# tumaer/lagrangebench

Measured on AMD Instinct MI355X. Metric: rollout particle-steps/sec, higher is better.
Workload: dtype f32 (GEMMs as fp16 hi/lo split products, fp32 accumulate)

## Files before the change

### lagrangebench_amd/build.py

```python
from __future__ import annotations

import os
import subprocess
import sys
from concurrent.futures import ThreadPoolExecutor

HERE = os.path.dirname(os.path.abspath(__file__))
CSRC = os.path.join(HERE, "csrc")
LIB = os.path.join(CSRC, "liblbhip.so")
SOURCES = ["lb_api.hip", "lb_neighbor.hip", "lb_state.hip", "lb_gns.hip", "lb_gns_weights.hip", "lb_edge16.hip", "lb_segnn.hip", "lb_segnn_gen.hip", "lb_segnn_msg.hip", "lb_segnn_node.hip", "lb_sinkhorn.hip", "lb_edge16v.hip", "lb_edge16w.hip", "lb_node16s.hip", "lb_gns_generic.hip", "lb_msplit.hip", "lb_train.hip", "lb_egnn.hip", "lb_painn.hip", "lb_train_input.hip"]
HEADERS = ["lb_internal.h", "lb_device.h", "lb_f16x2.h", "lb_segnn_dev.h", "lb_features.h", "lb_msplit.h", "lb_msplit_dev.h", "lb_lin32.h", "lb_train_segnn.h", "lb_train_egnn.h", os.path.join("..", "..", "include", "lbhip.h")]
FLAGS = ["-O3", "-std=c++17", "--offload-arch=gfx950", "-fPIC", "-ffp-contract=off",
         "-Wall", "-Wno-unused-function"]
EXTRA_FLAGS = {"lb_edge16v.hip": ["-fno-slp-vectorize"],
               "lb_edge16w.hip": ["-fno-slp-vectorize", "-mllvm", "-pragma-unroll-threshold=10000000"], "lb_node16s.hip": ["-fno-slp-vectorize"],
               "lb_gns_generic.hip": ["-fno-slp-vectorize"], "lb_segnn_msg.hip": ["-fno-slp-vectorize"], "lb_segnn_node.hip": ["-fno-slp-vectorize"], "lb_msplit.hip": ["-fno-slp-vectorize"]}


def _rocm_root() -> str:
    root = os.environ.get("ROCM_PATH")
    if root and os.path.isdir(root):
        return root
    try:
        out = subprocess.run(["hipconfig", "--rocmpath"], capture_output=True, text=True, timeout=30).stdout.strip()
        if out and os.path.isdir(out):
            return out
    except (OSError, subprocess.SubprocessError):
        pass
    return "/opt/rocm"


def _hipcc() -> str:
    for c in (os.path.join(_rocm_root(), "bin", "hipcc"), "/opt/rocm/bin/hipcc", "hipcc"):
        if os.path.exists(c) or c == "hipcc":
            return c
    raise RuntimeError("hipcc not found")


def _stale(target: str, deps) -> bool:
    if not os.path.exists(target):
        return True
    t = os.path.getmtime(target)
    return any(os.path.getmtime(d) > t for d in deps)

# ... 33 lines not shown
```

### lagrangebench_amd/csrc/lb_api.hip

```cpp
#include <cstddef>
#include <stdarg.h>
#include <stdio.h>
#include <stdlib.h>
#include <string.h>

#include <algorithm>
#include <cmath>

#include <initializer_list>
#include <tuple>

#include "lb_internal.h"
#include "lb_msplit.h"

thread_local std::string g_lb_err;

int lb_fail(int code, const char* fmt, ...) {
  char buf[1024];
  va_list ap;
  va_start(ap, fmt);
  vsnprintf(buf, sizeof(buf), fmt, ap);
  va_end(ap);
  g_lb_err = buf;
  return code;
// ... 85 lines not shown
  return (cls >= 0 && cls < LB_T_COUNT) ? k_timer_names[cls] : "";
}
extern "C" int lb_timer_get(lb_engine* e, int32_t cls, double* ms_out, int64_t* launches_out) {
  if (!e || cls < 0 || cls >= LB_T_COUNT) return lb_fail(LB_ERR_ARG, "bad timer class");
  lb_timers_collect(e);
  if (ms_out) *ms_out = e->t_ms[cls];
  if (launches_out) *launches_out = e->t_n[cls];
  return LB_OK;
}


extern "C" int lb_engine_create(const lb_case_desc* d, void* hip_stream, lb_engine** out) {
  if (!d || !out) return lb_fail(LB_ERR_ARG, "null argument");
  if (d->dim != 2 && d->dim != 3) return lb_fail(LB_ERR_ARG, "dim must be 2 or 3 (got %d)", d->dim);
  if (d->n_particles < 1 || d->batch < 1 || d->isl < 2)
    return lb_fail(LB_ERR_ARG, "need n_particles>=1, batch>=1, isl>=2");
  if (!(d->r_cutoff > 0)) return lb_fail(LB_ERR_ARG, "r_cutoff must be > 0");
  if ((int64_t)d->n_particles * d->batch > (int64_t)1 << 30)
    return lb_fail(LB_ERR_ARG, "B*N too large for int32 node ids");
  lb_engine* e = new lb_engine();
  e->desc = *d;
  e->stream = (hipStream_t)hip_stream;
  e->BN = (int64_t)d->n_particles * d->batch;
  e->timers_on = false;
  for (int i = 0; i < LB_T_COUNT; ++i) e->t_ms[i] = 0, e->t_n[i] = 0;
  {
    const char* f = getenv("LB_FUSED_AGG");
    e->fused_agg = (f && f[0] == '0') ? 0 : 1;
    const char* m = getenv("LB_MATH");
    e->f16x2 = (m && !strcmp(m, "f32")) ? 0 : 1;
    e->math_auto = m ? 0 : 1;
    const char* gf = getenv("LB_GUARD");
    e->guard_full = (gf && !strcmp(gf, "full")) ? 1 : 0;
    e->guard_sampled = (gf && !strcmp(gf, "sampled")) ? 1 : 0;
  }
  lb_geom& g = e->g;
  memset(&g, 0, sizeof(g));
  g.dim = d->dim;
  g.N = d->n_particles;
  g.B = d->batch;
  g.isl = d->isl;
  g.periodic = d->periodic != 0;
  g.has_bound = d->has_bound != 0;
  g.has_vel_mag = d->has_vel_mag != 0;
  g.force_kind = d->force_kind;
  g.force_axis = d->force_axis;
  g.f32 = d->geometry_f32 != 0;
  auto R = [&](double x) { return g.f32 ? (double)(float)x : x; };
  g.rc = R(d->r_cutoff);
  g.rc2 = R(d->r_cutoff * d->r_cutoff);
  bool use_cells = true;
  for (int k = 0; k < d->dim; ++k) {
    const float b32 = (float)d->box[k];
    if (!((float)d->r_cutoff < b32 / 3.0f)) use_cells = false;
  }
  g.use_cell_list = use_cells;
  g.ncells = 1;
  for (int k = 0; k < 3; ++k) {
    g.ncell[k] = 1;
    g.cell_size[k] = 1.0;
    g.box[k] = k < d->dim ? R(d->box[k]) : 1.0;
    g.half_box[k] = g.box[k] * 0.5;
    g.vel_mean[k] = R(d->vel_mean[k]);
    g.vel_std[k] = R(d->vel_std[k]);
    g.acc_mean[k] = R(d->acc_mean[k]);
    g.acc_std[k] = R(d->acc_std[k]);
// ... 698 lines not shown
```

### lagrangebench_amd/csrc/lb_gns.hip

```cpp
#include <stdio.h>

#include <algorithm>
#include <stdlib.h>

#include "lb_device.h"
#include "lb_msplit.h"

#define MFMA(a, b, c) __builtin_amdgcn_mfma_f32_32x32x2f32((a), (b), (c), 0, 0, 0)

void lb_pack_weight(const float* w, int K, int M, int Kpad, int Mpad, float* out) {
  const int NKQ = Kpad / 8, NMB = Mpad / 32;
  for (int kq = 0; kq < NKQ; ++kq)
    for (int mb = 0; mb < NMB; ++mb)
      for (int lane = 0; lane < 64; ++lane)
        for (int j = 0; j < 4; ++j) {
          const int k = 8 * kq + 4 * (lane >> 5) + j;
          const int m = 32 * mb + (lane & 31);
          out[(((size_t)kq * NMB + mb) * 64 + lane) * 4 + j] =
              (k < K && m < M) ? w[(size_t)k * M + m] : 0.f;
        }
}

template <int NKQ, int NMB, int PF = 1, typename LD>
__device__ __forceinline__ void lb_gemm(LD ld, const f32x4 (&v)[NKQ], f32x16 (&acc)[NMB]) {
// ... 300 lines not shown
    a.tile_shift = 4;
    a.row_ptr = e->row_ptr;
    a.part = e->part;
    if (ms) {
      lb_nms_args m{};
      m.ctrl = e->ctrl;
      m.n_rows = BN;
      m.xin = xin;
      m.agg = e->agg;
      m.row_ptr = e->row_ptr;
      m.part = e->part;
      m.fused = e->fused_agg;
      m.nlat = e->nlat;
      m.w = w.ms;
      m.b0 = a.b0;
      m.b1 = a.b1;
      m.ln_s = a.ln_s;
      m.ln_o = a.ln_o;
      m.bp = a.bp;
      m.psr = e->psr;
      if (dec) {
        m.bd0 = g->dec.b0;
        m.bd1 = g->dec.b1;
        m.dec_unscale = g->dec_unscale;
        m.acc_out = e->acc;
        m.out_dim = g->desc.out_dim;
        if (e->integ_job.on && g->desc.out_dim == e->g.dim) {
          m.integ = e->integ_job;
          e->integ_done = true;
        }
      }
      return lbk_node_ms(e, m, kq / 4, with_agg, resid, proj, dec);
    }
    if (e->f16x2)
      return lbk_node16s(e, a, w.w0_16h, w.w1_16h, proj ? g->proc_edge[next].proj_w_h2 : nullptr, kq / 4, with_agg ? 4 : 0,
                         resid);
    if (with_agg)
      hipLaunchKernelGGL((k_node_mlp<16, 16, true>), dim3(ntile_n), dim3(64), 0, s, a);
    else if (kq == 4)
      hipLaunchKernelGGL((k_node_mlp<4, 0, false>), dim3(ntile_n), dim3(64), 0, s, a);
    else if (kq == 8)
      hipLaunchKernelGGL((k_node_mlp<8, 0, false>), dim3(ntile_n), dim3(64), 0, s, a);
    else if (kq == 12)
      hipLaunchKernelGGL((k_node_mlp<12, 0, false>), dim3(ntile_n), dim3(64), 0, s, a);
    else
      hipLaunchKernelGGL((k_node_mlp<16, 0, false>), dim3(ntile_n), dim3(64), 0, s, a);
    return LB_OK;
  };

  lb_tic(e, LB_T_ENC_NODE);
  rc = node_mlp(g->enc_node, e->xnode, g->kq_node, false, false, 0, ms_en);
  lb_toc(e);
  if (rc) return rc;

  bool decoded = false;
  lb_tic(e, LB_T_ENC_EDGE);
  if (ms_ee) {
    lb_ems_args m{};
    m.ctrl = e->ctrl;
    m.efeat = e->efeat;
    m.elat = e->elat;
    m.w = g->enc_edge.ms;
    m.b0 = g->enc_edge.b0;
    m.b1 = g->enc_edge.b1;
    m.ln_s = g->enc_edge.ln_s;
    m.ln_o = g->enc_edge.ln_o;
    rc = lbk_edge_enc_ms(e, m);
  } else {
    lb_edge16_args b{};
// ... 34 lines not shown
    } else {
      lb_edge16_args b{};
      b.ctrl = e->ctrl;
      b.senders = e->senders;
      b.receivers = e->receivers;
      b.elat = e->elat;
      b.msg = e->msg;
      b.psr = e->psr;
      b.w0p = e->f16x2 ? pe.w0_16h : pe.w0_16;
      b.w1p = e->f16x2 ? pe.w1_16h : pe.w1_16;
      b.b1 = pe.b1;
      b.ln_s = pe.ln_s;
      b.ln_o = pe.ln_o;
      b.fused = e->fused_agg;
      b.row_ptr = e->row_ptr;
      b.agg = e->agg;
      b.part = e->part;
      b.aggpart_bytes = e->aggpart_bytes;
      b.skip_elat_store = skip;
      if (e->f16x2 && e->fused_agg)
        rc = lb_use_edge_w(e) ? lbk_edge16w(e, b) : lbk_edge16v(e, b);
      else
        rc = lbk_edge16(e, b, true, e->f16x2 != 0);
    }
    lb_toc(e);
    if (rc) return rc;
    if (!e->fused_agg) {
      lb_tic(e, LB_T_AGGREGATE);
      rc = lbk_segment_sum(e, e->msg, e->agg, LB_D);
      lb_toc(e);
      if (rc) return rc;
    }
    const bool ms_dec_ok = lb_fused_launches();
    const bool with_dec = ms_pn && ms_dec_ok && k == L - 1 && e->f16x2 && g->desc.out_dim <= 4;
    lb_tic_single(e, LB_T_NODE_MLP);
    rc = node_mlp(g->proc_node[k], e->nlat, 16, true, true, k + 1, ms_pn, with_dec);
    lb_toc(e);
    decoded = with_dec;
    if (rc) return rc;
    if (g->tap)
      LB_HIP(hipMemcpyAsync(g->tap + (size_t)(k + 1) * BN * LB_D, e->nlat, sizeof(float) * BN * LB_D,
                            hipMemcpyDeviceToDevice, s));
  }
  if (decoded) return LB_OK;
  lb_tic(e, LB_T_DECODER);
  rc = lbk_decoder16(e, g);
  lb_toc(e);
  if (rc) return rc;
  LB_HIP(hipGetLastError());
  return LB_OK;
}
```

### lagrangebench_amd/csrc/lb_gns_generic.hip

```cpp
#include <algorithm>
#include <cmath>
#include <cstring>
#include <vector>

#include "lb_f16x2.h"
#include "lb_features.h"

#define MFMA16F(a, b, c) __builtin_amdgcn_mfma_f32_16x16x4f32((a), (b), (c), 0, 0, 0)
#define GD_THREADS 512
#define GD_WAVES 8

struct lb_dense_args {
  const lb_ctrl* ctrl;
  int64_t n_rows;
  const float* x;
  int x_blocked;
  int x_stride, x_width;
  const float* w;
  const float* bias;
  const float* add0;
  const int32_t* idx0;
  const float* add1;
  const int32_t* idx1;
  const float* ln_s;
  const float* ln_o;
  const float* resid;
  int resid_blocked;
  float* out;
  int out_blocked;
  float* out_pre;
  float* acc_out;
  int out_dim;
};

__device__ __forceinline__ void lb_gemm16f(lds_cptr wl, const f32x4 (&v)[8], f32x4 (&acc)[8]) {
  f32x4 a0 = wl[0], a1 = wl[64];
#pragma unroll
  for (int step = 0; step < 32; ++step) {
    f32x4 n0 = a0, n1 = a1;
// ... 125 lines not shown
      bool bad = false;
      for (int d = 0; d < a.out_dim; ++d) bad |= !(fabsf(o[d]) <= 3.0e38f);
      if (bad) lb_raise_math(a.ctrl, LB_MATH_NONFINITE);
    }
  }
}

static int lbk_dense16(lb_engine* e, const lb_dense_args& a, int64_t rows_bound, bool relu_in) {
  const int64_t tiles = std::max<int64_t>(1, (rows_bound + 15) / 16);
  const int grid = (int)std::min<int64_t>(512, (tiles + GD_WAVES - 1) / GD_WAVES);
  if (e->f16x2) {
    if (relu_in)
      hipLaunchKernelGGL((k_dense16<true, true>), dim3(grid), dim3(GD_THREADS), 0, e->stream, a);
    else
      hipLaunchKernelGGL((k_dense16<true, false>), dim3(grid), dim3(GD_THREADS), 0, e->stream, a);
  } else {
    if (relu_in)
      hipLaunchKernelGGL((k_dense16<false, true>), dim3(grid), dim3(GD_THREADS), 0, e->stream, a);
    else
      hipLaunchKernelGGL((k_dense16<false, false>), dim3(grid), dim3(GD_THREADS), 0, e->stream, a);
  }
  LB_HIP(hipGetLastError());
  return LB_OK;
}

struct lb_dec16_args {
  const lb_ctrl* ctrl;
  int64_t n_rows;
  const float* nlat;
  const float* w0;
  const float* b0;
  const float* w1;
  const float* b1;
  float unscale;
  float* acc_out;
  int out_dim;
  lb_integ_job integ;
};

template <bool F16>
__global__ void __launch_bounds__(GD_THREADS, 2) k_decoder16(lb_dec16_args a, lb_geom geom) {
  constexpr int NW1 = F16 ? 512 : 4096;
  __shared__ f32x4 sW[4096 + NW1 + 33];
  const int poisoned = a.ctrl->overflow_step;
  const int step = a.ctrl->step;
  const int tid = threadIdx.x;
  {
    const f32x4* g0 = reinterpret_cast<const f32x4*>(a.w0);
    const f32x4* g1 = reinterpret_cast<const f32x4*>(a.w1);
    for (int i = tid; i < 4096; i += GD_THREADS) sW[i] = g0[i];
    for (int i = tid; i < NW1; i += GD_THREADS) sW[4096 + i] = g1[i];
    if (tid < 32) sW[4096 + NW1 + tid] = reinterpret_cast<const f32x4*>(a.b0)[tid];
    if (tid == 32) sW[4096 + NW1 + 32] = reinterpret_cast<const f32x4*>(a.b1)[0];
  }
  if (poisoned >= 0) return;
  __syncthreads();
  const int ntiles = (int)((a.n_rows + 15) >> 4);
  const int lane = tid & 63, wave = tid >> 6;
  const int n = lane & 15, g = lane >> 4;
  const lds_cptr lw0 = (lds_cptr)sW + lane, lw1 = (lds_cptr)sW + 4096 + lane;
  const lds_cptr lb0 = (lds_cptr)sW + 4096 + NW1 + g;
  const f32x4 b1v = sW[4096 + NW1 + 32];
  const f32x4 zero = {0.f, 0.f, 0.f, 0.f};
  bool probed = false;
  for (int t = blockIdx.x * GD_WAVES + wave; t < ntiles; t += gridDim.x * GD_WAVES) {
    const int64_t row = (int64_t)t * 16 + n;
    const bool valid = row < a.n_rows;
    const int64_t rowc = valid ? row : a.n_rows - 1;
    f32x4 v[8], acc[8];
    lb_integ_in pre{};
    if (a.integ.on && valid && g == 0) pre = lb_integrate_fetch(geom, a.n_rows, a.integ.win, step, a.integ.ptype, row);
    const f32x4* xr = reinterpret_cast<const f32x4*>(a.nlat) + rowc * 32 + g;
#pragma unroll
    for (int mb = 0; mb < 8; ++mb) v[mb] = xr[4 * mb];
#pragma unroll
    for (int mb = 0; mb < 8; ++mb) acc[mb] = lb0[4 * mb];
    f32x4 o = zero;
    if constexpr (F16) {
      if (!probed) {
        lb_range_probe(a.ctrl, v, 8);
        probed = true;
      }
      lb_gemm16v<false, 4>(lw0, v, acc);
      if (t < (int)gridDim.x * GD_WAVES) lb_range_probe(a.ctrl, acc, 8);
#pragma unroll
      for (int p = 0; p < 4; ++p) {
        f32x4 r0, r1;
#pragma unroll
        for (int j = 0; j < 4; ++j) {
          r0[j] = fmaxf(acc[2 * p][j], 0.f);
          r1[j] = fmaxf(acc[2 * p + 1][j], 0.f);
        }
        h8 bh, bl;
        lb_split8v(r0, r1, bh, bl);
        const h8 ah = __builtin_bit_cast(h8, lw1[(p * 2 + 0) * 64]);
        const h8 al = __builtin_bit_cast(h8, lw1[(p * 2 + 1) * 64]);
        o = MFMA16H(al, bh, o);
        o = MFMA16H(ah, bl, o);
        o = MFMA16H(ah, bh, o);
      }
    } else {
      lb_gemm16f(lw0, v, acc);
#pragma unroll
      for (int step = 0; step < 32; ++step) {
        const f32x4 a0 = lw1[(step * 2) * 64];
        o = MFMA16F(a0[0], fmaxf(acc[step >> 2][step & 3], 0.f), o);
      }
    }
    if (valid && g == 0) {
      o = o * a.unscale + b1v;
      reinterpret_cast<f32x4*>(a.acc_out)[row] = o;
      bool bad = false;
      for (int d = 0; d < a.out_dim; ++d) bad |= !(fabsf(o[d]) <= 3.0e38f);
      if (bad) lb_raise_math(a.ctrl, LB_MATH_NONFINITE);
      if (a.integ.on) {
        const float av[4] = {o[0], o[1], o[2], o[3]};
        lb_integrate_body(geom, a.n_rows, a.integ.win, step, a.integ.ptype, av, nullptr, a.integ.traj, a.integ.T,
                          a.integ.pred, a.integ.pred_T, row, &pre);
      }
    }
  }
  if (a.integ.on) {
    __syncthreads();
    if (tid == 0 && atomicAdd(a.integ.blocks_done, 1) == (int)gridDim.x - 1) {
      *a.integ.blocks_done = 0;
      const_cast<lb_ctrl*>(a.ctrl)->step = step + 1;
    }
  }
}

int lbk_decoder16(lb_engine* e, lb_gns* g) {
  lb_dec16_args a{};
  a.ctrl = e->ctrl;
  a.n_rows = e->BN;
  a.nlat = e->nlat;
  a.w0 = e->f16x2 ? g->dec.w0_16h : g->dec.w0_16;
  a.b0 = g->dec.b0;
  a.w1 = e->f16x2 ? g->dec.w1_16h : g->dec.w1_16;
  a.b1 = g->dec.b1;
  a.unscale = e->f16x2 ? g->dec_unscale : 1.f;
  a.acc_out = e->acc;
  a.out_dim = g->desc.out_dim;
  const int64_t tiles = std::max<int64_t>(1, (e->BN + 15) / 16);
  const int grid = (int)std::min<int64_t>(512, (tiles + GD_WAVES - 1) / GD_WAVES);
  if (e->integ_job.on && g->desc.out_dim == e->g.dim) {
    a.integ = e->integ_job;
    e->integ_done = true;
  }
  if (e->f16x2)
    hipLaunchKernelGGL((k_decoder16<true>), dim3(grid), dim3(GD_THREADS), 0, e->stream, a, e->g);
  else
    hipLaunchKernelGGL((k_decoder16<false>), dim3(grid), dim3(GD_THREADS), 0, e->stream, a, e->g);
  LB_HIP(hipGetLastError());
  return LB_OK;
}

int lbk_gns_forward_generic(lb_engine* e, lb_gns* g) {
  hipStream_t s = e->stream;
  const int64_t BN = e->BN;
  const int D = LB_D, L = g->desc.num_mp_steps, nl = g->desc.blocks_per_step;
  int rc;
  if (nl > 1 && g->gen_he_cap < e->e_alloc) {
    LB_HIP(hipStreamSynchronize(s));
    if (g->gen_he) (void)hipFree(g->gen_he);
    g->gen_he = nullptr;
    g->gen_he_cap = 0;
    LB_TRY(lb_alloc(&g->gen_he, (size_t)(e->e_alloc + 32) * D));
    g->gen_he_cap = e->e_alloc;
  }
  const int64_t e_bound = e->e_alloc;
  auto W = [&](const lb_gen_lin& l, int blk) { return e->f16x2 ? l.wh[blk] : l.wf[blk]; };
  auto base_args = [&]() {
    lb_dense_args a{};
    a.ctrl = e->ctrl;
    a.x_stride = D;
    a.x_width = D;
    a.out_dim = g->desc.out_dim;
    return a;
  };
// ... 172 lines not shown
```

### lagrangebench_amd/csrc/lb_gns_weights.hip

```cpp
#include <algorithm>
#include <cmath>
#include <cstdio>
#include <cstring>
#include <utility>
#include <vector>

#include "lb_msplit.h"

struct lb_lin_view {
  const float* w;
  int blocks, rows, out;
  const float* b;
  const float* block(int i) const { return w + (size_t)i * rows * out; }
};
struct lb_mlp_view {
  std::vector<lb_lin_view> lin;
  const float* ln_s = nullptr;
  const float* ln_o = nullptr;
};
struct lb_gns_view {
  const float* embed = nullptr;
  lb_mlp_view enc_node, enc_edge, dec;
  std::vector<lb_mlp_view> proc_edge, proc_node;
};
// ... 165 lines not shown
    put_ms(&m.ms, ms);
  };
  auto proj_piece = [&](const std::vector<float>& wsr) { return std::vector<ms_piece>{{wsr.data(), D, 2 * D, 4, 2, true, 0}}; };

  std::vector<float> wsr, wsr_next;
  if (L) wsr = ws_wr(v.proc_edge[0].lin[0]);
  node_mlp(g->enc_node, v.enc_node, v.enc_node.lin[0].w, v.enc_node.lin[0].rows, dl, g->kq_node * 8,
           L ? proj_piece(wsr) : std::vector<ms_piece>());
  g->proc_edge.resize(L);
  g->proc_node.resize(L);
  for (int k = 0; k < L; ++k) {
    {
      const lb_lin_view &l0 = v.proc_edge[k].lin[0], &l1 = v.proc_edge[k].lin[1];
      lb_mlp_w& m = g->proc_edge[k];
      p32(&m.proj_w, wsr.data(), D, 2 * D, D, 2 * D);
      float* two = st.put(&m.proj_w_h2, (size_t)2 * D * D);
      lb_pack_weight16h(l0.block(0), dl, dl, D, two, D);
      lb_pack_weight16h(l0.block(1), dl, dl, D, two + (size_t)D * D, D);
      memcpy(st.put(&m.proj_b, 2 * D) + D, l0.b, sizeof(float) * dl);
      p16(&m.w0_16, l0.block(2), dl, dl, D);
      p16h(&m.w0_16h, l0.block(2), dl, dl, D);
      p16(&m.w1_16, l1.w, dl, dl, D);
      p16h(&m.w1_16h, l1.w, dl, dl, D);
      vecs(m, v.proc_edge[k], false);
      put_ms(&m.ms, {{l0.block(2), dl, dl, 4, 1, true, 0}, {l1.w, dl, dl, 4, 1, true, 0}});
    }
    const std::vector<float> w0 = lb_lin_padded(v.proc_node[k].lin[0]);
    std::vector<ms_piece> ms = {{d0.w, dl, dl, 4, 1, true, 0}, {d1s.data(), dl, od, 4, 1, true, 2048}};
    if (k + 1 < L) {
      wsr_next = ws_wr(v.proc_edge[k + 1].lin[0]);
      ms = proj_piece(wsr_next);
    }
    node_mlp(g->proc_node[k], v.proc_node[k], w0.data(), 2 * D, D, 2 * D, ms);
    wsr.swap(wsr_next);
  }
}

static void lb_pack_dense(lb_stage& st, const lb_gns_view& v, lb_gns* g) {
  const int D = LB_D, L = g->desc.num_mp_steps;
  auto mlp = [&](lb_gen_mlp& m, const lb_mlp_view& s) {
    m.lin.resize(s.lin.size());
    for (size_t li = 0; li < s.lin.size(); ++li) {
      const lb_lin_view& l = s.lin[li];
      lb_gen_lin& x = m.lin[li];
      st.note_rms(l);
      x.wh.resize(l.blocks);
      x.wf.resize(l.blocks);
      for (int b = 0; b < l.blocks; ++b) {
        lb_pack_weight16h(l.block(b), l.rows, l.out, D, st.put(&x.wh[b], (size_t)D * D), D);
        lb_pack_weight16(l.block(b), l.rows, l.out, D, st.put(&x.wf[b], (size_t)D * D));
      }
      st.put(&x.b, D, l.b, l.out);
    }
    if (s.ln_s) {
      st.put(&m.ln_s, D, s.ln_s, s.lin.back().out);
      st.put(&m.ln_o, D, s.ln_o, s.lin.back().out);
    }
  };
  mlp(g->g_enc_node, v.enc_node);
  mlp(g->g_enc_edge, v.enc_edge);
  g->g_proc_edge.resize(L);
  g->g_proc_node.resize(L);
  for (int k = 0; k < L; ++k) {
    mlp(g->g_proc_edge[k], v.proc_edge[k]);
    mlp(g->g_proc_node[k], v.proc_node[k]);
  }
// ... 73 lines not shown
```

### lagrangebench_amd/csrc/lb_internal.h

```cpp
#pragma once
#include <cstdlib>
#include <hip/hip_ext.h>
#include <hip/hip_runtime.h>
#include <stdint.h>

#include <string>
#include <vector>

#include "../../include/lbhip.h"

#define LB_MAX_STENCIL_CAND 2048
#define LB_MAX_ROW 256
#define LB_MAX_ROW_DENSE 4096
#define LB_TILE 32
#define LB_D 128
#define LB_PAD_TYPE (-1)

typedef float f32x4 __attribute__((ext_vector_type(4)));
typedef float f32x16 __attribute__((ext_vector_type(16)));

struct lb_ctrl {
  int32_t step;
  int32_t overflow_step;
  int32_t n_edges_total;
// ... 116 lines not shown
  unsigned long long* nl_wg_sum = nullptr;
  int32_t* row_ptr;
  int32_t* scan_part;
  double* cpos;
  int64_t cell_slots = 0;
  bool nl_dense = false;
  int32_t row_cap = 0;
  int32_t maxd;
  int32_t* tmp_send;
  float* tmp_feat;
  double* tmp_feat64;
  int32_t* senders;
  int32_t* receivers;
  float* efeat;
  double* efeat64;
  int32_t* overflow;
  int32_t* nedges_b;

  float* xnode;
  float* nlat;
  float* agg;
  float* psr;
  float* elat;
  float* msg;
  float* part;
  int64_t aggpart_bytes = 0;
  int fused_agg;
  int f16x2;
  int math_auto;
  int guard_sampled;
  int math_fallbacks = 0;
  int debug_guard_step = -1;
  int debug_guard_flags = 0;
  int guard_full;
  float* acc;
  const void* bound_model = nullptr;

  bool timers_on;
  std::vector<lb_timer_rec> trecs;
  bool ext_armed = false, ext_used = false;
  std::vector<hipEvent_t> epool;
  double t_ms[LB_T_COUNT];
  int64_t t_n[LB_T_COUNT];
};

struct lb_mlp_w {
  const float* b0;
  const float* b1;
  const float* ln_s;
  const float* ln_o;
  const float* w0;
  const float* w1;
  const float* w0_16;
  const float* w1_16;
  const float* w0_16h;
  const float* w1_16h;
  const float* ms;
  const float* proj_w;
  const float* proj_w_h2;
  const float* proj_b;
};

struct lb_edge16_args {
  const lb_ctrl* ctrl;
  const int32_t* senders;
  const int32_t* receivers;
  const float* efeat;
  float* elat;
  float* elat_out;
  float* msg;
  const float* psr;
  const float* w0p;
  const float* b0;
  const float* w1p;
  const float* b1;
  const float* ln_s;
  const float* ln_o;
  int fused;
  const int32_t* row_ptr;
  float* agg;
  float* part;
  int64_t aggpart_bytes;
  int reverse;
  int skip_elat_store;
};

struct lb_node_args {
  const lb_ctrl* ctrl;
  int64_t n_rows;
  const float* xin;
  const float* agg;
  float* nlat;
  const float* w0p;
// ... 142 lines not shown
int lbk_sgg_forward(lb_engine* e, lb_sgg* m);

void lb_sg_msg_image(const float* ws0, const float* wv0, const float* b0, const float* ws1,
                     const float* wv1, const float* b1, float* out);
int lb_sg_msg_image_floats(void);
int lbk_sg_message(lb_engine* e, const float* f, const float* image, float* agg, float* part, int64_t out_bytes,
                   bool finish);
void lb_sg_upd_image(const float* ws0, const float* wv0, const float* b0, const float* ws1,
                     const float* wv1, const float* b1, float* out);
int lb_sg_upd_image_floats(void);
int lbk_sg_update(lb_engine* e, float* f, const float* agg, const float* part, const float* nattr, const float* image,
                  bool combine_partials);

void lb_sg_embed_image(const float* ws, const float* wv, const float* b, int ns, int nv, float* out);
int lb_sg_embed_image_floats(void);
int lbk_sg_embed(lb_engine* e, const float* xnode, const float* image, float* f, float* nattr, int homogeneous,
                 int vel_avg);
void lb_sg_readout_image(const float* ws0, const float* wv0, const float* b0, const float* ws1, const float* wv1,
                         const float* b1, const float* wo, float* out);
int lb_sg_readout_image_floats(void);
int lbk_sg_readout(lb_engine* e, const float* f, const float* nattr, const float* image, float* acc_out);

int lb_ensure_node_scratch(lb_engine* e);
int lb_gns_bind(lb_engine* e, lb_gns* g);
int lbk_gns_forward(lb_engine* e, lb_gns* g);
int lbk_gns_forward_generic(lb_engine* e, lb_gns* g);
int lbk_decoder16(lb_engine* e, lb_gns* g);
int lbk_segment_sum(lb_engine* e, const float* msg, float* out, int D);
void lb_pack_weight(const float* w, int K, int M, int Kpad, int Mpad, float* out);

void lb_pack_weight16(const float* w, int K, int M, int Kpad, float* out);
void lb_pack_weight16h(const float* w, int K, int M, int Kpad, float* out, int Mpad = 128);

int lbk_node16s(lb_engine* e, const lb_node_args& a, const float* w0h, const float* w1h,
                const float* wph2, int npa, int npb, bool resid);
int lbk_edge16(lb_engine* e, const lb_edge16_args& a, bool proc, bool f16x2);
int lbk_edge16v(lb_engine* e, const lb_edge16_args& a);
int lbk_edge16w(lb_engine* e, const lb_edge16_args& a);
int lbk_edge_enc16v(lb_engine* e, const lb_edge16_args& a);
```

### lagrangebench_amd/csrc/lb_node16s.hip

```cpp
#include <stdlib.h>

#include "lb_f16x2.h"

#define NS_CHUNK 2048

typedef __attribute__((address_space(3))) f32x4* lds_ptr;
typedef const __attribute__((address_space(1))) void* gbl_cvptr;

template <int MB0>
__device__ __forceinline__ void lb_load_agg_half(const lb_node_args& a, int64_t gnode, int g, int k0, int k1,
                                                 f32x4 (&v)[4]) {
  if (!a.fused) {
    const f32x4* gr = reinterpret_cast<const f32x4*>(a.agg) + gnode * 32 + g;
#pragma unroll
    for (int mb = 0; mb < 4; ++mb) v[mb] = gr[4 * (MB0 + mb)];
#pragma unroll
    for (int mb = 0; mb < 4; ++mb) asm volatile("" : "+v"(v[mb]));
    return;
  }
  const int t0 = k0 >> a.tile_shift, t1 = (k1 - 1) >> a.tile_shift;
  const bool single = t0 == t1;
  const int nsrc = (k1 <= k0) ? 0 : (single ? 1 : t1 - t0 + 1);
#pragma unroll
  for (int mb = 0; mb < 4; ++mb) v[mb] = f32x4{0.f, 0.f, 0.f, 0.f};
  for (int s = 0; __any(s < nsrc); ++s) {
    if (s < nsrc) {
      const int t = t0 + s;
      const float* src = single ? a.agg + gnode * 128
                                : a.part + ((int64_t)t * 2 + (k0 <= (t << a.tile_shift) ? 0 : 1)) * 128;
      const f32x4* s4 = reinterpret_cast<const f32x4*>(src) + g;
#pragma unroll
      for (int mb = 0; mb < 4; ++mb) v[mb] = v[mb] + s4[4 * (MB0 + mb)];
    }
  }
}

template <int NPA, int NPB, bool RESID, bool PROJ, int NW, int NS_SLOTS>
__global__ void __launch_bounds__(NW * 64, NW == 4 ? (NS_SLOTS == 4 ? 1 : 2) : 4)
    k_node16s(lb_node_args a, const f32x4* __restrict__ w0h, const f32x4* __restrict__ w1h,
              const f32x4* __restrict__ wph) {
  __shared__ f32x4 sB[NS_SLOTS][NS_CHUNK];
  __shared__ f32x4 sP[192];
  if (a.ctrl->overflow_step >= 0) return;
  const int tid = threadIdx.x, lane = tid & 63, wave = __builtin_amdgcn_readfirstlane(tid >> 6);
  const int n = lane & 15, g = lane >> 4;
  constexpr int NP0 = NPA + NPB;
  constexpr int NCH0 = (NP0 + 1) / 2;
  constexpr int n_chunks = NCH0 + 2 + (PROJ ? 4 : 0);
  static_assert(NPB == 0 || (NPA == 4 && NPB == 4), "processor shape: 4 + 4 k-steps");

  if (tid < 128) {
    const float* src = tid < 32 ? a.b0 : (tid < 64 ? a.b1 : (tid < 96 ? a.ln_s : a.ln_o));
    sP[tid] = reinterpret_cast<const f32x4*>(src)[tid & 31];
  } else if (tid < 192) {
    sP[tid] = (PROJ && a.bp) ? reinterpret_cast<const f32x4*>(a.bp)[tid - 128] : f32x4{0.f, 0.f, 0.f, 0.f};
  }

  auto issue_chunk = [&](int c) {
    const f32x4* src;
    int nvec = NS_CHUNK;
    if (c < NCH0) {
      src = w0h + (size_t)c * NS_CHUNK;
      if (2 * c + 2 > NP0) nvec = NS_CHUNK / 2;
    } else if (c < NCH0 + 2) {
      src = w1h + (size_t)(c - NCH0) * NS_CHUNK;
    } else {
      src = wph + (size_t)(c - NCH0 - 2) * NS_CHUNK;
    }
    f32x4* slot = sB[c % NS_SLOTS];
#pragma unroll
    for (int i = 0; i < 32 / NW; ++i) {
      const int piece = wave + NW * i;
      if (piece * 64 < nvec) {
        const uint32_t voff = (uint32_t)(piece * 64 + lane) * 16u;
        const uint32_t lo = (uint32_t)(uintptr_t)(lds_ptr)(slot + piece * 64);
        asm volatile("s_mov_b32 m0, %2\n\tglobal_load_lds_dwordx4 %0, %1" ::"v"(voff), "s"(src), "s"(lo) : "memory");
      }
    }
  };
  constexpr int DPC = 32 / NW;
#define NS_STEP(c)                                                                     \
  do {                                                                                 \
    constexpr int later = ((c) + NS_SLOTS - 2 < n_chunks ? NS_SLOTS - 2 : n_chunks - 1 - (c)); \
    if constexpr (later * DPC == 0) asm volatile("s_waitcnt vmcnt(0)" ::: "memory");   \
    if constexpr (later * DPC == 1) asm volatile("s_waitcnt vmcnt(1)" ::: "memory");   \
    if constexpr (later * DPC == 2) asm volatile("s_waitcnt vmcnt(2)" ::: "memory");   \
    if constexpr (later * DPC == 4) asm volatile("s_waitcnt vmcnt(4)" ::: "memory");   \
    if constexpr (later * DPC == 8) asm volatile("s_waitcnt vmcnt(8)" ::: "memory");   \
    if constexpr (later * DPC == 16) asm volatile("s_waitcnt vmcnt(16)" ::: "memory"); \
    if constexpr ((c) == 0) {                                                          \
      __syncthreads();                \
    } else {                                                                           \
      asm volatile("s_waitcnt lgkmcnt(0)\n\ts_barrier" ::: "memory");                  \
    }                                                                                  \
  } while (0)
#define NS_REFILL(c)                                                           \
  do {                                                                         \
    if constexpr ((c) >= 1 && (c)-1 + NS_SLOTS < n_chunks) issue_chunk((c)-1 + NS_SLOTS); \
  } while (0)
#pragma unroll
// ... 64 lines not shown
  NS_REFILL(C1);
#pragma unroll
  for (int mb = 0; mb < 8; ++mb) acc2[mb] = vecp[32 + 4 * mb];
  {
    const f32x4 v01[4] = {acc[0], acc[1], acc[2], acc[3]};
    uint32_t or_h = 0;
    lb_gemm16v<true, 2, 1>(NS_BUF(C1), v01, acc2, &or_h);
    if (lb_rows_tiny(or_h) && lane == 0) lb_raise_math(a.ctrl, LB_MATH_TINY);
  }
  NS_STEP(C1 + 1);
  f32x4 res[8];
  if constexpr (RESID) {
    const f32x4* xr = reinterpret_cast<const f32x4*>(a.xin) + rowc * 32 + g;
#pragma unroll
    for (int mb = 0; mb < 4; ++mb) res[mb] = xr[4 * mb];
  }
  NS_REFILL(C1 + 1);
  {
    const f32x4 v23[4] = {acc[4], acc[5], acc[6], acc[7]};
    lb_gemm16v<true, 2>(NS_BUF(C1 + 1), v23, acc2);
  }
  if constexpr (RESID) {
    const f32x4* xr = reinterpret_cast<const f32x4*>(a.xin) + rowc * 32 + g;
#pragma unroll
    for (int mb = 4; mb < 8; ++mb) res[mb] = xr[4 * mb];
  }
  f32x4 y[8];
  lb_layernorm16(acc2, vecp + 64, vecp + 96, y, a.ctrl->ln_inv_d, a.ctrl->ln_pad);
  if constexpr (RESID) {
#pragma unroll
    for (int mb = 0; mb < 8; ++mb) y[mb] = lb_pk_add(res[mb], y[mb]);
  }
  if (probe) lb_range_probe(a.ctrl, y, 8);
  if (valid) {
    f32x4* nr = reinterpret_cast<f32x4*>(a.nlat) + row * 32 + g;
#pragma unroll
    for (int mb = 0; mb < 8; ++mb) nr[4 * mb] = y[mb];
  }
  if constexpr (PROJ) {
    {
      f32x4 accp[8];
      NS_STEP(CP);
      NS_REFILL(CP);
#pragma unroll
      for (int mb = 0; mb < 8; ++mb) accp[mb] = vecp[128 + 4 * mb];
      {
        const f32x4 v01[4] = {y[0], y[1], y[2], y[3]};
        lb_gemm16v<false, 2>(NS_BUF(CP), v01, accp);
      }
      NS_STEP(CP + 1);
      NS_REFILL(CP + 1);
      {
        const f32x4 v23[4] = {y[4], y[5], y[6], y[7]};
        lb_gemm16v<false, 2>(NS_BUF(CP + 1), v23, accp);
      }
      if (valid) {
        f32x4* pr = reinterpret_cast<f32x4*>(a.psr) + row * 64 + g;
#pragma unroll
        for (int mb = 0; mb < 8; ++mb) pr[4 * mb] = accp[mb];
      }
    }
    {
      f32x4 accp[8];
      NS_STEP(CP + 2);
      NS_REFILL(CP + 2);
#pragma unroll
      for (int mb = 0; mb < 8; ++mb) accp[mb] = vecp[128 + 32 + 4 * mb];
      {
        const f32x4 v01[4] = {y[0], y[1], y[2], y[3]};
        lb_gemm16v<false, 2>(NS_BUF(CP + 2), v01, accp);
      }
      NS_STEP(CP + 3);
      NS_REFILL(CP + 3);
      {
        const f32x4 v23[4] = {y[4], y[5], y[6], y[7]};
        lb_gemm16v<false, 2>(NS_BUF(CP + 3), v23, accp);
      }
      if (valid) {
        f32x4* pr = reinterpret_cast<f32x4*>(a.psr) + row * 64 + 32 + g;
#pragma unroll
        for (int mb = 0; mb < 8; ++mb) pr[4 * mb] = accp[mb];
      }
    }
  }
#undef NS_BUF
}
#undef NS_STEP
#undef NS_REFILL


int lbk_node16s(lb_engine* e, const lb_node_args& a, const float* w0h, const float* w1h, const float* wph2,
                int npa, int npb, bool resid) {
  const f32x4* w0 = reinterpret_cast<const f32x4*>(w0h);
  const f32x4* w1 = reinterpret_cast<const f32x4*>(w1h);
  const f32x4* wp = reinterpret_cast<const f32x4*>(wph2);
  const bool proj = wph2 != nullptr;
  const int64_t tiles = (a.n_rows + 15) / 16;
  const int nw = tiles < 8 * 256 ? 4 : 8;
  const int nblk = (int)((tiles + nw - 1) / nw);
  dim3 grid(nblk), block(nw * 64);
#define LB_NS(A, B, R, P, W, S) \
  LB_LAUNCH_TIMED(e, (k_node16s<A, B, R, P, W, S>), grid, block, a, w0, w1, wp)
#define LB_NS_W(A, B, R, P)            \
  do {                                 \
    if (nw == 8)                       \
      LB_NS(A, B, R, P, 8, 2);         \
    else                               \
      LB_NS(A, B, R, P, 4, 2);         \
  } while (0)
#define LB_NS_P(A, B, R)               \
  do {                                 \
    if (proj)                          \
      LB_NS_W(A, B, R, true);          \
    else                               \
      LB_NS_W(A, B, R, false);         \
  } while (0)
  if (npa == 4 && npb == 4 && resid)
    LB_NS_P(4, 4, true);
  else if (npa == 1 && npb == 0 && !resid)
    LB_NS_P(1, 0, false);
  else if (npa == 2 && npb == 0 && !resid)
    LB_NS_P(2, 0, false);
  else if (npa == 3 && npb == 0 && !resid)
    LB_NS_P(3, 0, false);
  else if (npa == 4 && npb == 0 && !resid)
    LB_NS_P(4, 0, false);
  else
    return lb_fail(LB_ERR_UNSUPPORTED, "k_node16s<%d,%d,%d> not instantiated", npa, npb, (int)resid);
  LB_HIP(hipGetLastError());
  return LB_OK;
}
```

Baseline: 20.87 million.

## Fuse GNS decoder MLP and integration into last processor node kernel

Adds a DEC variant of the f16x2 node kernel that, for the final processor layer, runs the two-layer decoder head and the integration step directly on the in-register node latents instead of writing them to global memory. A separate decoder launch is dropped, along with the round trip of node latents through memory. Decoder weights are pre-packed per last layer and streamed through the existing shared-memory chunk ring with a short final chunk. In exchange the kernel uses more registers and LDS traffic, and it adds a grid-wide completion counter to advance the step.

```diff
diff --git a/lagrangebench_amd/build.py b/lagrangebench_amd/build.py
--- a/lagrangebench_amd/build.py
+++ b/lagrangebench_amd/build.py
@@ -9,7 +9,7 @@
 CSRC = os.path.join(HERE, "csrc")
 LIB = os.path.join(CSRC, "liblbhip.so")
 SOURCES = ["lb_api.hip", "lb_neighbor.hip", "lb_state.hip", "lb_gns.hip", "lb_gns_weights.hip", "lb_edge16.hip", "lb_segnn.hip", "lb_segnn_gen.hip", "lb_segnn_msg.hip", "lb_segnn_node.hip", "lb_sinkhorn.hip", "lb_edge16v.hip", "lb_edge16w.hip", "lb_node16s.hip", "lb_gns_generic.hip", "lb_msplit.hip", "lb_train.hip", "lb_egnn.hip", "lb_painn.hip", "lb_train_input.hip"]
-HEADERS = ["lb_internal.h", "lb_device.h", "lb_f16x2.h", "lb_segnn_dev.h", "lb_features.h", "lb_msplit.h", "lb_msplit_dev.h", "lb_lin32.h", "lb_train_segnn.h", "lb_train_egnn.h", os.path.join("..", "..", "include", "lbhip.h")]
+HEADERS = ["lb_internal.h", "lb_device.h", "lb_f16x2.h", "lb_dec16.h", "lb_segnn_dev.h", "lb_features.h", "lb_msplit.h", "lb_msplit_dev.h", "lb_lin32.h", "lb_train_segnn.h", "lb_train_egnn.h", os.path.join("..", "..", "include", "lbhip.h")]
 FLAGS = ["-O3", "-std=c++17", "--offload-arch=gfx950", "-fPIC", "-ffp-contract=off",
          "-Wall", "-Wno-unused-function"]
 EXTRA_FLAGS = {"lb_edge16v.hip": ["-fno-slp-vectorize"],
diff --git a/lagrangebench_amd/csrc/lb_api.hip b/lagrangebench_amd/csrc/lb_api.hip
--- a/lagrangebench_amd/csrc/lb_api.hip
+++ b/lagrangebench_amd/csrc/lb_api.hip
@@ -141,6 +141,8 @@
     e->math_auto = m ? 0 : 1;
     const char* gf = getenv("LB_GUARD");
     e->guard_full = (gf && !strcmp(gf, "full")) ? 1 : 0;
+    const char* bd = getenv("LB_BATCH_FUSED_DEC");
+    e->batch_fused_dec = (bd && bd[0] == '0') ? 0 : 1;
     e->guard_sampled = (gf && !strcmp(gf, "sampled")) ? 1 : 0;
   }
   lb_geom& g = e->g;
diff --git a/lagrangebench_amd/csrc/lb_dec16.h b/lagrangebench_amd/csrc/lb_dec16.h
--- /dev/null
+++ b/lagrangebench_amd/csrc/lb_dec16.h
@@ -0,0 +1,56 @@
+#pragma once
+#include "lb_f16x2.h"
+#include "lb_features.h"
+
+struct lb_dec16_out {
+  float unscale;
+  float* acc_out;
+  int out_dim;
+  lb_integ_job integ;
+};
+
+__device__ __forceinline__ f32x4 lb_dec16_head(const f32x4 (&hid)[8], lds_cptr lw1) {
+  f32x4 o = {0.f, 0.f, 0.f, 0.f};
+#pragma unroll
+  for (int p = 0; p < 4; ++p) {
+    f32x4 r0, r1;
+#pragma unroll
+    for (int j = 0; j < 4; ++j) {
+      r0[j] = fmaxf(hid[2 * p][j], 0.f);
+      r1[j] = fmaxf(hid[2 * p + 1][j], 0.f);
+    }
+    h8 bh, bl;
+    lb_split8v(r0, r1, bh, bl);
+    const h8 ah = __builtin_bit_cast(h8, lw1[(p * 2 + 0) * 64]);
+    const h8 al = __builtin_bit_cast(h8, lw1[(p * 2 + 1) * 64]);
+    o = MFMA16H(al, bh, o);
+    o = MFMA16H(ah, bl, o);
+    o = MFMA16H(ah, bh, o);
+  }
+  return o;
+}
+
+__device__ __forceinline__ void lb_dec16_finish(const lb_ctrl* ctrl, const lb_dec16_out& a, const lb_geom& geom,
+                                                int64_t n_rows, int step, f32x4 o, const f32x4& b1v, int64_t row,
+                                                const lb_integ_in* pre) {
+  o = o * a.unscale + b1v;
+  reinterpret_cast<f32x4*>(a.acc_out)[row] = o;
+  bool bad = false;
+  for (int d = 0; d < a.out_dim; ++d) bad |= !(fabsf(o[d]) <= 3.0e38f);
+  if (bad) lb_raise_math(ctrl, LB_MATH_NONFINITE);
+  if (a.integ.on) {
+    const float av[4] = {o[0], o[1], o[2], o[3]};
+    lb_integrate_body(geom, n_rows, a.integ.win, step, a.integ.ptype, av, nullptr, a.integ.traj, a.integ.T, a.integ.pred,
+                      a.integ.pred_T, row, pre);
+  }
+}
+
+__device__ __forceinline__ void lb_dec16_advance(const lb_ctrl* ctrl, const lb_dec16_out& a, int step) {
+  if (a.integ.on) {
+    __syncthreads();
+    if (threadIdx.x == 0 && atomicAdd(a.integ.blocks_done, 1) == (int)gridDim.x - 1) {
+      *a.integ.blocks_done = 0;
+      const_cast<lb_ctrl*>(ctrl)->step = step + 1;
+    }
+  }
+}
diff --git a/lagrangebench_amd/csrc/lb_gns.hip b/lagrangebench_amd/csrc/lb_gns.hip
--- a/lagrangebench_amd/csrc/lb_gns.hip
+++ b/lagrangebench_amd/csrc/lb_gns.hip
@@ -356,9 +356,23 @@
       }
       return lbk_node_ms(e, m, kq / 4, with_agg, resid, proj, dec);
     }
-    if (e->f16x2)
+    if (e->f16x2) {
+      lb_node16s_dec nd{};
+      if (dec) {
+        nd.w_16h = w.dec_16h;
+        nd.b0 = g->dec.b0;
+        nd.b1 = g->dec.b1;
+        nd.unscale = g->dec_unscale;
+        nd.acc_out = e->acc;
+        nd.out_dim = g->desc.out_dim;
+        if (e->integ_job.on && g->desc.out_dim == e->g.dim) {
+          nd.integ = e->integ_job;
+          e->integ_done = true;
+        }
+      }
       return lbk_node16s(e, a, w.w0_16h, w.w1_16h, proj ? g->proc_edge[next].proj_w_h2 : nullptr, kq / 4, with_agg ? 4 : 0,
-                         resid);
+                         resid, dec ? &nd : nullptr);
+    }
     if (with_agg)
       hipLaunchKernelGGL((k_node_mlp<16, 16, true>), dim3(ntile_n), dim3(64), 0, s, a);
     else if (kq == 4)
@@ -459,7 +473,8 @@
       if (rc) return rc;
     }
     const bool ms_dec_ok = lb_fused_launches();
-    const bool with_dec = ms_pn && ms_dec_ok && k == L - 1 && e->f16x2 && g->desc.out_dim <= 4;
+    const bool tail_ok = k == L - 1 && e->f16x2 && g->desc.out_dim <= 4;
+    const bool with_dec = tail_ok && (ms_pn ? ms_dec_ok : (e->batch_fused_dec && !g->tap));
     lb_tic_single(e, LB_T_NODE_MLP);
     rc = node_mlp(g->proc_node[k], e->nlat, 16, true, true, k + 1, ms_pn, with_dec);
     lb_toc(e);
diff --git a/lagrangebench_amd/csrc/lb_gns_generic.hip b/lagrangebench_amd/csrc/lb_gns_generic.hip
--- a/lagrangebench_amd/csrc/lb_gns_generic.hip
+++ b/lagrangebench_amd/csrc/lb_gns_generic.hip
@@ -3,8 +3,7 @@
 #include <cstring>
 #include <vector>
 
-#include "lb_f16x2.h"
-#include "lb_features.h"
+#include "lb_dec16.h"
 
 #define MFMA16F(a, b, c) __builtin_amdgcn_mfma_f32_16x16x4f32((a), (b), (c), 0, 0, 0)
 #define GD_THREADS 512
@@ -196,10 +195,7 @@
   const float* b0;
   const float* w1;
   const float* b1;
-  float unscale;
-  float* acc_out;
-  int out_dim;
-  lb_integ_job integ;
+  lb_dec16_out out;
 };
 
 template <bool F16>
@@ -233,7 +229,8 @@
     const int64_t rowc = valid ? row : a.n_rows - 1;
     f32x4 v[8], acc[8];
     lb_integ_in pre{};
-    if (a.integ.on && valid && g == 0) pre = lb_integrate_fetch(geom, a.n_rows, a.integ.win, step, a.integ.ptype, row);
+    if (a.out.integ.on && valid && g == 0)
+      pre = lb_integrate_fetch(geom, a.n_rows, a.out.integ.win, step, a.out.integ.ptype, row);
     const f32x4* xr = reinterpret_cast<const f32x4*>(a.nlat) + rowc * 32 + g;
 #pragma unroll
     for (int mb = 0; mb < 8; ++mb) v[mb] = xr[4 * mb];
@@ -247,22 +244,7 @@
       }
       lb_gemm16v<false, 4>(lw0, v, acc);
       if (t < (int)gridDim.x * GD_WAVES) lb_range_probe(a.ctrl, acc, 8);
-#pragma unroll
-      for (int p = 0; p < 4; ++p) {
-        f32x4 r0, r1;
-#pragma unroll
-        for (int j = 0; j < 4; ++j) {
-          r0[j] = fmaxf(acc[2 * p][j], 0.f);
-          r1[j] = fmaxf(acc[2 * p + 1][j], 0.f);
-        }
-        h8 bh, bl;
-        lb_split8v(r0, r1, bh, bl);
-        const h8 ah = __builtin_bit_cast(h8, lw1[(p * 2 + 0) * 64]);
-        const h8 al = __builtin_bit_cast(h8, lw1[(p * 2 + 1) * 64]);
-        o = MFMA16H(al, bh, o);
-        o = MFMA16H(ah, bl, o);
-        o = MFMA16H(ah, bh, o);
-      }
+      o = lb_dec16_head(acc, lw1);
     } else {
       lb_gemm16f(lw0, v, acc);
 #pragma unroll
@@ -271,26 +253,9 @@
         o = MFMA16F(a0[0], fmaxf(acc[step >> 2][step & 3], 0.f), o);
       }
     }
-    if (valid && g == 0) {
-      o = o * a.unscale + b1v;
-      reinterpret_cast<f32x4*>(a.acc_out)[row] = o;
-      bool bad = false;
-      for (int d = 0; d < a.out_dim; ++d) bad |= !(fabsf(o[d]) <= 3.0e38f);
-      if (bad) lb_raise_math(a.ctrl, LB_MATH_NONFINITE);
-      if (a.integ.on) {
-        const float av[4] = {o[0], o[1], o[2], o[3]};
-        lb_integrate_body(geom, a.n_rows, a.integ.win, step, a.integ.ptype, av, nullptr, a.integ.traj, a.integ.T,
-                          a.integ.pred, a.integ.pred_T, row, &pre);
-      }
-    }
-  }
-  if (a.integ.on) {
-    __syncthreads();
-    if (tid == 0 && atomicAdd(a.integ.blocks_done, 1) == (int)gridDim.x - 1) {
-      *a.integ.blocks_done = 0;
-      const_cast<lb_ctrl*>(a.ctrl)->step = step + 1;
-    }
-  }
+    if (valid && g == 0) lb_dec16_finish(a.ctrl, a.out, geom, a.n_rows, step, o, b1v, row, &pre);
+  }
+  lb_dec16_advance(a.ctrl, a.out, step);
 }
 
 int lbk_decoder16(lb_engine* e, lb_gns* g) {
@@ -302,13 +267,13 @@
   a.b0 = g->dec.b0;
   a.w1 = e->f16x2 ? g->dec.w1_16h : g->dec.w1_16;
   a.b1 = g->dec.b1;
-  a.unscale = e->f16x2 ? g->dec_unscale : 1.f;
-  a.acc_out = e->acc;
-  a.out_dim = g->desc.out_dim;
+  a.out.unscale = e->f16x2 ? g->dec_unscale : 1.f;
+  a.out.acc_out = e->acc;
+  a.out.out_dim = g->desc.out_dim;
   const int64_t tiles = std::max<int64_t>(1, (e->BN + 15) / 16);
   const int grid = (int)std::min<int64_t>(512, (tiles + GD_WAVES - 1) / GD_WAVES);
   if (e->integ_job.on && g->desc.out_dim == e->g.dim) {
-    a.integ = e->integ_job;
+    a.out.integ = e->integ_job;
     e->integ_done = true;
   }
   if (e->f16x2)
diff --git a/lagrangebench_amd/csrc/lb_gns_weights.hip b/lagrangebench_amd/csrc/lb_gns_weights.hip
--- a/lagrangebench_amd/csrc/lb_gns_weights.hip
+++ b/lagrangebench_amd/csrc/lb_gns_weights.hip
@@ -221,6 +221,11 @@
       ms = proj_piece(wsr_next);
     }
     node_mlp(g->proc_node[k], v.proc_node[k], w0.data(), 2 * D, D, 2 * D, ms);
+    if (k + 1 == L) {
+      float* tail = st.put(&g->proc_node[k].dec_16h, (size_t)D * D + (size_t)D * 16);
+      lb_pack_weight16h(d0.w, dl, dl, D, tail, D);
+      lb_pack_weight16h(d1s.data(), dl, od, D, tail + (size_t)D * D, 16);
+    }
     wsr.swap(wsr_next);
   }
 }
diff --git a/lagrangebench_amd/csrc/lb_internal.h b/lagrangebench_amd/csrc/lb_internal.h
--- a/lagrangebench_amd/csrc/lb_internal.h
+++ b/lagrangebench_amd/csrc/lb_internal.h
@@ -172,6 +172,7 @@
   int math_fallbacks = 0;
   int debug_guard_step = -1;
   int debug_guard_flags = 0;
+  int batch_fused_dec;
   int guard_full;
   float* acc;
   const void* bound_model = nullptr;
@@ -199,6 +200,7 @@
   const float* proj_w;
   const float* proj_w_h2;
   const float* proj_b;
+  const float* dec_16h;
 };
 
 struct lb_edge16_args {
@@ -407,8 +409,17 @@
 void lb_pack_weight16(const float* w, int K, int M, int Kpad, float* out);
 void lb_pack_weight16h(const float* w, int K, int M, int Kpad, float* out, int Mpad = 128);
 
+struct lb_node16s_dec {
+  const float* w_16h;
+  const float* b0;
+  const float* b1;
+  float unscale;
+  float* acc_out;
+  int out_dim;
+  lb_integ_job integ;
+};
 int lbk_node16s(lb_engine* e, const lb_node_args& a, const float* w0h, const float* w1h,
-                const float* wph2, int npa, int npb, bool resid);
+                const float* wph2, int npa, int npb, bool resid, const lb_node16s_dec* dec = nullptr);
 int lbk_edge16(lb_engine* e, const lb_edge16_args& a, bool proc, bool f16x2);
 int lbk_edge16v(lb_engine* e, const lb_edge16_args& a);
 int lbk_edge16w(lb_engine* e, const lb_edge16_args& a);
diff --git a/lagrangebench_amd/csrc/lb_node16s.hip b/lagrangebench_amd/csrc/lb_node16s.hip
--- a/lagrangebench_amd/csrc/lb_node16s.hip
+++ b/lagrangebench_amd/csrc/lb_node16s.hip
@@ -1,6 +1,6 @@
 #include <stdlib.h>
 
-#include "lb_f16x2.h"
+#include "lb_dec16.h"
 
 #define NS_CHUNK 2048
 
@@ -35,25 +35,37 @@
   }
 }
 
-template <int NPA, int NPB, bool RESID, bool PROJ, int NW, int NS_SLOTS>
+struct lb_node_dec {
+  const float* b0;
+  const float* b1;
+  lb_dec16_out out;
+  lb_geom geom;
+};
+template <int NPA, int NPB, bool RESID, bool PROJ, int NW, int NS_SLOTS, bool DEC = false>
 __global__ void __launch_bounds__(NW * 64, NW == 4 ? (NS_SLOTS == 4 ? 1 : 2) : 4)
     k_node16s(lb_node_args a, const f32x4* __restrict__ w0h, const f32x4* __restrict__ w1h,
-              const f32x4* __restrict__ wph) {
+              const f32x4* __restrict__ wph, lb_node_dec d) {
   __shared__ f32x4 sB[NS_SLOTS][NS_CHUNK];
   __shared__ f32x4 sP[192];
+  static_assert(!DEC || (!PROJ && NS_SLOTS == 2), "decoder variant: last layer, two-slot ring (its last chunk is a short one)");
   if (a.ctrl->overflow_step >= 0) return;
+  const int step = DEC ? a.ctrl->step : 0;
   const int tid = threadIdx.x, lane = tid & 63, wave = __builtin_amdgcn_readfirstlane(tid >> 6);
   const int n = lane & 15, g = lane >> 4;
   constexpr int NP0 = NPA + NPB;
   constexpr int NCH0 = (NP0 + 1) / 2;
-  constexpr int n_chunks = NCH0 + 2 + (PROJ ? 4 : 0);
+  constexpr int n_chunks = NCH0 + 2 + (PROJ ? 4 : 0) + (DEC ? 3 : 0);
   static_assert(NPB == 0 || (NPA == 4 && NPB == 4), "processor shape: 4 + 4 k-steps");
 
   if (tid < 128) {
     const float* src = tid < 32 ? a.b0 : (tid < 64 ? a.b1 : (tid < 96 ? a.ln_s : a.ln_o));
     sP[tid] = reinterpret_cast<const f32x4*>(src)[tid & 31];
   } else if (tid < 192) {
-    sP[tid] = (PROJ && a.bp) ? reinterpret_cast<const f32x4*>(a.bp)[tid - 128] : f32x4{0.f, 0.f, 0.f, 0.f};
+    if constexpr (DEC) {
+      if (tid <= 160) sP[tid] = tid < 160 ? reinterpret_cast<const f32x4*>(d.b0)[tid - 128] : reinterpret_cast<const f32x4*>(d.b1)[0];
+    } else {
+      sP[tid] = (PROJ && a.bp) ? reinterpret_cast<const f32x4*>(a.bp)[tid - 128] : f32x4{0.f, 0.f, 0.f, 0.f};
+    }
   }
 
   auto issue_chunk = [&](int c) {
@@ -66,6 +78,7 @@
       src = w1h + (size_t)(c - NCH0) * NS_CHUNK;
     } else {
       src = wph + (size_t)(c - NCH0 - 2) * NS_CHUNK;
+      if (DEC && c == n_chunks - 1) nvec = NS_CHUNK / 4;
     }
     f32x4* slot = sB[c % NS_SLOTS];
 #pragma unroll
@@ -196,7 +209,7 @@
     for (int mb = 0; mb < 8; ++mb) y[mb] = lb_pk_add(res[mb], y[mb]);
   }
   if (probe) lb_range_probe(a.ctrl, y, 8);
-  if (valid) {
+  if (valid && !DEC) {
     f32x4* nr = reinterpret_cast<f32x4*>(a.nlat) + row * 32 + g;
 #pragma unroll
     for (int mb = 0; mb < 8; ++mb) nr[4 * mb] = y[mb];
@@ -247,6 +260,31 @@
       }
     }
   }
+  if constexpr (DEC) {
+    f32x4 hid[8];
+    NS_STEP(CP);
+    NS_REFILL(CP);
+#pragma unroll
+    for (int mb = 0; mb < 8; ++mb) hid[mb] = vecp[128 + 4 * mb];
+    {
+      const f32x4 v01[4] = {y[0], y[1], y[2], y[3]};
+      lb_gemm16v<false, 2>(NS_BUF(CP), v01, hid);
+    }
+    NS_STEP(CP + 1);
+    NS_REFILL(CP + 1);
+    {
+      const f32x4 v23[4] = {y[4], y[5], y[6], y[7]};
+      lb_gemm16v<false, 2>(NS_BUF(CP + 1), v23, hid);
+    }
+    lb_integ_in pre{};
+    if (d.out.integ.on && valid && g == 0)
+      pre = lb_integrate_fetch(d.geom, a.n_rows, d.out.integ.win, step, d.out.integ.ptype, row);
+    if (probe) lb_range_probe(a.ctrl, hid, 8);
+    NS_STEP(CP + 2);
+    const f32x4 o = lb_dec16_head(hid, NS_BUF(CP + 2));
+    if (valid && g == 0) lb_dec16_finish(a.ctrl, d.out, d.geom, a.n_rows, step, o, sP[160], row, &pre);
+    lb_dec16_advance(a.ctrl, d.out, step);
+  }
 #undef NS_BUF
 }
 #undef NS_STEP
@@ -254,17 +292,29 @@
 
 
 int lbk_node16s(lb_engine* e, const lb_node_args& a, const float* w0h, const float* w1h, const float* wph2,
-                int npa, int npb, bool resid) {
+                int npa, int npb, bool resid, const lb_node16s_dec* dec) {
   const f32x4* w0 = reinterpret_cast<const f32x4*>(w0h);
   const f32x4* w1 = reinterpret_cast<const f32x4*>(w1h);
-  const f32x4* wp = reinterpret_cast<const f32x4*>(wph2);
+  const f32x4* wp = reinterpret_cast<const f32x4*>(dec ? dec->w_16h : wph2);
   const bool proj = wph2 != nullptr;
+  lb_node_dec d{};
+  if (dec) {
+    if (proj || !(npa == 4 && npb == 4 && resid))
+      return lb_fail(LB_ERR_UNSUPPORTED, "k_node16s<DEC>: last processor layer only");
+    d.b0 = dec->b0;
+    d.b1 = dec->b1;
+    d.out.unscale = dec->unscale;
+    d.out.acc_out = dec->acc_out;
+    d.out.out_dim = dec->out_dim;
+    d.out.integ = dec->integ;
+    d.geom = e->g;
+  }
   const int64_t tiles = (a.n_rows + 15) / 16;
   const int nw = tiles < 8 * 256 ? 4 : 8;
   const int nblk = (int)((tiles + nw - 1) / nw);
   dim3 grid(nblk), block(nw * 64);
 #define LB_NS(A, B, R, P, W, S) \
-  LB_LAUNCH_TIMED(e, (k_node16s<A, B, R, P, W, S>), grid, block, a, w0, w1, wp)
+  LB_LAUNCH_TIMED(e, (k_node16s<A, B, R, P, W, S>), grid, block, a, w0, w1, wp, d)
 #define LB_NS_W(A, B, R, P)            \
   do {                                 \
     if (nw == 8)                       \
@@ -279,7 +329,12 @@
     else                               \
       LB_NS_W(A, B, R, false);         \
   } while (0)
-  if (npa == 4 && npb == 4 && resid)
+  if (dec) {
+    if (nw == 8)
+      LB_LAUNCH_TIMED(e, (k_node16s<4, 4, true, false, 8, 2, true>), grid, block, a, w0, w1, wp, d);
+    else
+      LB_LAUNCH_TIMED(e, (k_node16s<4, 4, true, false, 4, 2, true>), grid, block, a, w0, w1, wp, d);
+  } else if (npa == 4 && npb == 4 && resid)
     LB_NS_P(4, 4, true);
   else if (npa == 1 && npb == 0 && !resid)
     LB_NS_P(1, 0, false);
```

Result: no change. 20.96 million, median of 6 (+0.4%).
